# xingyizhou/CenterTrack

Hardware: AMD Instinct MI355X
Metric: frames/sec (DLA-34 + DCNv2 CenterTrack hot path: H2D of the frame + forward + decode + D2H + track association) (higher is better)
Workload: dtype f32; 1 GPU; mot17_512: mot heads, DLA-34, 512x512, 1 stream(s)/GPU, K=100, flip_test=False, seeded random-init weights; one step = 64 consecutive frames of every stream, each frame uploaded from pinned host memory inside the step (frame t+1 on a copy stream while frame t runs); global_batch=1, parallelism=streams sharded dp1, all-gather of packed detections, hip_graph=True

## Files before the change

centertrack_amd/csrc/frame_loop.hip:

```cpp
#include <stdlib.h>
#include <string.h>
#include <time.h>

#include <atomic>
#include <condition_variable>
#include <mutex>
#include <thread>
#include <vector>

#include "ct_common.h"

namespace {

class StreamPool {
public:
    explicit StreamPool(int helpers) {
        for (int i = 0; i < helpers; ++i) th_.emplace_back([this] { worker(); });
    }
    ~StreamPool() {
        {
            std::lock_guard<std::mutex> g(m_);
            stop_ = true;
            ++gen_;
        }
        cv_.notify_all();
        for (auto &t : th_) t.join();
    }
    bool run(int total, bool (*fn)(void *, int), void *ctx) {
        fn_ = fn; ctx_ = ctx; total_ = total; ok_.store(true);
        next_.store(0);
        pending_.store((int)th_.size());
        {
            std::lock_guard<std::mutex> g(m_);
            ++gen_;
        }
        cv_.notify_all();
        drain();
        while (pending_.load(std::memory_order_acquire) > 0) __builtin_ia32_pause();
        return ok_.load();
    }
private:
    void drain() {
        for (;;) {
            const int i = next_.fetch_add(1);
            if (i >= total_) break;
            if (!fn_(ctx_, i)) ok_.store(false);
        }
    }
    void worker() {
        unsigned seen = 0;
        for (;;) {
            {
                std::unique_lock<std::mutex> lk(m_);
                cv_.wait(lk, [&] { return gen_ != seen; });
                seen = gen_;
                if (stop_) return;
            }
            drain();
            pending_.fetch_sub(1, std::memory_order_release);
        }
    }
    std::vector<std::thread> th_;
    std::mutex m_;
    std::condition_variable cv_;
    unsigned gen_ = 0;
    bool stop_ = false;
    bool (*fn_)(void *, int) = nullptr;
    void *ctx_ = nullptr;
    int total_ = 0;
    std::atomic<int> next_{0}, pending_{0};
    std::atomic<bool> ok_{true};
};

struct Loop {
    ct_frame_loop_desc d;
    hipStream_t copy_stream = nullptr;
    hipEvent_t frame_ready = nullptr;
    hipEvent_t frame_done = nullptr;
    int uploaded_slot = -1;
    int pre_done_slot = -1;
    bool in_flight = false;
    int flight_slot = -1;
    StreamPool *pool = nullptr;
    ~Loop() { delete pool; }
};

struct AssocJob {
    const ct_frame_loop_desc *d;
    const float *rows, *trans_inv;
    int *counts;
    std::atomic<int> failed{-1};
    char err[256] = {0};
};

bool assoc_one(void *ctx, int b)
{
    AssocJob &j = *(AssocJob *)ctx;
    const ct_frame_loop_desc &d = *j.d;
    const int n = ct_tracker_step(d.trackers[b], j.rows + (size_t)b * d.K * d.F, d.K, d.F, &d.layout, d.out_thresh,
                                  j.trans_inv + 6 * b, d.results + (size_t)b * d.results_cap, d.results_cap);
    j.counts[b] = n;
    if (n < 0) {
        int none = -1;
        if (j.failed.compare_exchange_strong(none, b)) {
            strncpy(j.err, ct_last_error(), sizeof(j.err) - 1);
            j.err[sizeof(j.err) - 1] = 0;
        }
    }
    return n >= 0;
}

int fail(const char *what, hipError_t e)
{
    ct_set_error("%s: %s", what, hipGetErrorString(e));
    return CT_ERR_LAUNCH;
}

int prestage(Loop *L, int slot)
{
    const ct_frame_loop_desc &d = L->d;
    if (!d.pre.enabled || L->pre_done_slot == slot) return CT_OK;
    const ct_prestage_desc &p = d.pre;
    float *cur = d.frames[slot];
    const float *prev = d.frames[(slot + d.nslots - 1) % d.nslots];
    if (p.flip_B > 0) {
        const size_t half = (size_t)p.flip_B * 3 * p.H * p.W;
        int rc = ct_flip_images(cur, cur + half, (size_t)p.flip_B * 3 * p.H, p.W, d.stream);
        if (rc != CT_OK) return rc;
    }
    int rc = ct_stem_forward_parts(cur, prev, nullptr, nullptr, 0, p.N, p.H, p.W, p.w_x, p.w_img, nullptr, p.scale3, p.shift3,
                                   p.partial[slot], p.ldp, d.stream);
    if (rc != CT_OK) return rc;
    L->pre_done_slot = slot;
    return CT_OK;
}

}

extern "C" void *ct_frame_loop_create(const ct_frame_loop_desc *d)
{
    if (!d || d->B <= 0 || d->K <= 0 || d->F <= 0 || !d->trackers || !d->host_rows || !d->results || d->results_cap <= 0 ||
        d->nslots < 1 || d->nslots > 3 || d->frame_bytes == 0) {
        ct_set_error("ct_frame_loop_create: bad descriptor");
        return nullptr;
    }
    for (int i = 0; i < d->nslots; ++i)
        if (!d->graphs[i] || !d->frames[i]) {
            ct_set_error("ct_frame_loop_create: slot %d has no graph / frame buffer", i);
            return nullptr;
        }
    if (d->blob_params && (!d->blob_counts || d->blob_cap <= 0)) {
        ct_set_error("ct_frame_loop_create: blob_params without counts / capacity");
        return nullptr;
    }
    Loop *L = new Loop();
    L->d = *d;
    {
        const char *env = getenv("CENTERTRACK_HOST_THREADS");
        int threads = env ? atoi(env) : (d->B >= 8 ? (d->B / 4 < 8 ? d->B / 4 : 8) : 1);
        if (threads > d->B) threads = d->B;
        if (threads > 1) L->pool = new StreamPool(threads - 1);
    }
    hipError_t e = hipStreamCreateWithFlags(&L->copy_stream, hipStreamNonBlocking);
    if (e == hipSuccess) e = hipEventCreateWithFlags(&L->frame_ready, hipEventDisableTiming);
    if (e == hipSuccess) e = hipEventCreateWithFlags(&L->frame_done, hipEventDisableTiming);
    if (d->pre.enabled && (d->nslots != 3 || !d->pre.w_x || !d->pre.w_img || !d->pre.scale3 || !d->pre.shift3 ||
                           !d->pre.partial[0] || !d->pre.partial[1] || !d->pre.partial[2] || d->pre.ldp < 16)) {
        ct_set_error("ct_frame_loop_create: incomplete pre-stage description");
        e = hipErrorInvalidValue;
    }
    if (e != hipSuccess) {
        ct_set_error("ct_frame_loop_create: %s", hipGetErrorString(e));
        if (L->copy_stream) (void)hipStreamDestroy(L->copy_stream);
        delete L;
        return nullptr;
    }
    return L;
}

extern "C" void ct_frame_loop_destroy(void *loop)
{
    Loop *L = (Loop *)loop;
    if (!L) return;
    if (L->in_flight && L->frame_done) (void)hipEventSynchronize(L->frame_done);
    if (L->copy_stream) { (void)hipStreamSynchronize(L->copy_stream); (void)hipStreamDestroy(L->copy_stream); }
    if (L->frame_ready) (void)hipEventDestroy(L->frame_ready);
    if (L->frame_done) (void)hipEventDestroy(L->frame_done);
    delete L;
}

extern "C" int ct_frame_loop_pending_slot(void *loop) { return loop ? ((Loop *)loop)->uploaded_slot : -1; }

extern "C" int ct_frame_loop_in_flight(void *loop) { return (loop && ((Loop *)loop)->in_flight) ? ((Loop *)loop)->flight_slot : -1; }

extern "C" void ct_frame_loop_forget_upload(void *loop)
{
    Loop *L = (Loop *)loop;
    if (!L) return;
    if (L->uploaded_slot >= 0) (void)hipStreamSynchronize(L->copy_stream);
    L->uploaded_slot = -1;
    L->pre_done_slot = -1;
}

extern "C" int ct_frame_loop_prestage(void *loop, int slot)
{
    Loop *L = (Loop *)loop;
    if (!L) CT_FAIL_ARG("ct_frame_loop_prestage: null loop");
    if (slot < 0 || slot >= L->d.nslots) CT_FAIL_ARG("ct_frame_loop_prestage: slot %d of %d", slot, L->d.nslots);
    const int rc = prestage(L, slot);
    L->pre_done_slot = -1;
    return rc;
}

extern "C" int ct_frame_loop_submit(void *loop, const ct_frame_step_args *a)
{
    Loop *L = (Loop *)loop;
    if (!L || !a) CT_FAIL_ARG("ct_frame_loop_submit: null argument");
    const ct_frame_loop_desc &d = L->d;
    if (L->in_flight) CT_FAIL_ARG("ct_frame_loop_submit: the previous frame was not finished");
    if (a->slot < 0 || a->slot >= d.nslots) CT_FAIL_ARG("ct_frame_loop_submit: slot %d of %d", a->slot, d.nslots);
    hipStream_t s = (hipStream_t)d.stream;
    if (d.blob_params) {
        if (!a->trans_input) CT_FAIL_ARG("ct_frame_loop_submit: trans_input missing");
        for (int b = 0; b < d.B; ++b) {
            const int n = ct_tracker_prehm_params(d.trackers[b], d.pre_thresh, a->trans_input + 6 * b, d.inp_w, d.inp_h,
                                                  d.blob_params + (size_t)b * d.blob_cap * 3, d.blob_cap);
            if (n < 0) return CT_ERR_ARG;
            d.blob_counts[b] = n;
        }
    }
    hipError_t e = hipSuccess;
    if (a->frame_kind == CT_FRAME_UPLOADED) {
        if (L->uploaded_slot != a->slot) CT_FAIL_ARG("ct_frame_loop_submit: no upload pending for slot %d (pending: %d)", a->slot, L->uploaded_slot);
        e = hipStreamWaitEvent(s, L->frame_ready, 0);
        if (e != hipSuccess) return fail("ct_frame_loop_submit(wait for the uploaded frame)", e);
    } else if (a->frame_kind == CT_FRAME_DEVICE || a->frame_kind == CT_FRAME_HOST) {
        if (!a->frame) CT_FAIL_ARG("ct_frame_loop_submit: null frame");
        if (L->uploaded_slot >= 0) {
            e = hipStreamWaitEvent(s, L->frame_ready, 0);
            if (e != hipSuccess) return fail("ct_frame_loop_submit(wait for a stale upload)", e);
        }
        e = hipMemcpyAsync(d.frames[a->slot], a->frame, d.frame_bytes,
                           a->frame_kind == CT_FRAME_DEVICE ? hipMemcpyDeviceToDevice : hipMemcpyHostToDevice, s);
        if (e != hipSuccess) return fail("ct_frame_loop_submit(frame copy)", e);
    } else if (a->frame_kind != CT_FRAME_IN_PLACE) {
        CT_FAIL_ARG("ct_frame_loop_submit: frame_kind %d", a->frame_kind);
    }
    L->uploaded_slot = -1;
    if (a->frame_kind != CT_FRAME_UPLOADED && L->pre_done_slot == a->slot) L->pre_done_slot = -1;
    {
        const int rc = prestage(L, a->slot);
        if (rc != CT_OK) return rc;
        L->pre_done_slot = -1;
    }
    if (d.done_flag) __atomic_store_n(d.done_flag, 0, __ATOMIC_RELEASE);
    e = hipGraphLaunch((hipGraphExec_t)d.graphs[a->slot], s);
    if (e == hipSuccess) e = hipEventRecord(L->frame_done, s);
    if (e != hipSuccess) return fail("ct_frame_loop_submit(graph launch)", e);
    L->in_flight = true;
    L->flight_slot = a->slot;
    if (a->next_frame) {
        if (d.nslots < 2) CT_FAIL_ARG("ct_frame_loop_submit: uploading ahead needs >= 2 slots");
        const int ns = (a->slot + 1) % d.nslots;
        e = hipMemcpyAsync(d.frames[ns], a->next_frame, d.frame_bytes, hipMemcpyHostToDevice, L->copy_stream);
        if (e == hipSuccess) e = hipEventRecord(L->frame_ready, L->copy_stream);
        if (e != hipSuccess) return fail("ct_frame_loop_submit(upload of the next frame; the frame itself is in flight)", e);
        L->uploaded_slot = ns;
        if (d.pre.enabled) {
            e = hipStreamWaitEvent(s, L->frame_ready, 0);
            if (e != hipSuccess) return fail("ct_frame_loop_submit(pre-stage of the next frame)", e);
            const int rc = prestage(L, ns);
            if (rc != CT_OK) return rc;
        }
    }
    return CT_OK;
}

extern "C" int ct_frame_loop_upload(void *loop, int slot, const float *frame)
{
    Loop *L = (Loop *)loop;
    if (!L || !frame) CT_FAIL_ARG("ct_frame_loop_upload: null argument");
    const ct_frame_loop_desc &d = L->d;
    if (slot < 0 || slot >= d.nslots) CT_FAIL_ARG("ct_frame_loop_upload: slot %d of %d", slot, d.nslots);
    if (L->in_flight && (slot == L->flight_slot || (d.nslots == 3 && slot == (L->flight_slot + 2) % 3)))
        CT_FAIL_ARG("ct_frame_loop_upload: slot %d is read by the frame in flight", slot);
    hipError_t e = hipMemcpyAsync(d.frames[slot], frame, d.frame_bytes, hipMemcpyHostToDevice, L->copy_stream);
    if (e == hipSuccess) e = hipEventRecord(L->frame_ready, L->copy_stream);
    if (e != hipSuccess) return fail("ct_frame_loop_upload", e);
    L->uploaded_slot = slot;
    L->pre_done_slot = -1;
    if (d.pre.enabled && L->in_flight) {
        e = hipStreamWaitEvent((hipStream_t)d.stream, L->frame_ready, 0);
        if (e != hipSuccess) return fail("ct_frame_loop_upload(pre-stage)", e);
        const int rc = prestage(L, slot);
        if (rc != CT_OK) return rc;
    }
    return CT_OK;
}

extern "C" int ct_frame_loop_wait(void *loop)
{
    Loop *L = (Loop *)loop;
    if (!L) CT_FAIL_ARG("ct_frame_loop_wait: null loop");
    if (!L->in_flight) return CT_OK;
    bool seen = false;
    if (L->d.done_flag) {
        struct timespec t0, t1;
        clock_gettime(CLOCK_MONOTONIC, &t0);
        for (unsigned it = 0;; ++it) {
            if (__atomic_load_n(L->d.done_flag, __ATOMIC_ACQUIRE) == 1) { seen = true; break; }
            __builtin_ia32_pause();
            if ((it & 0x3ff) == 0x3ff) {
                clock_gettime(CLOCK_MONOTONIC, &t1);
                if ((t1.tv_sec - t0.tv_sec) * 1000000000L + (t1.tv_nsec - t0.tv_nsec) > 50000000L) break;
            }
        }
    }
    if (!seen) {
        hipError_t e = hipEventSynchronize(L->frame_done);
        if (e != hipSuccess) return fail("ct_frame_loop_wait", e);
    }
    L->in_flight = false;
    return CT_OK;
}

extern "C" int ct_frame_loop_finish(void *loop, const ct_frame_step_args *a, int *counts)
{
    Loop *L = (Loop *)loop;
    if (!L || !a || !counts) CT_FAIL_ARG("ct_frame_loop_finish: null argument");
    const ct_frame_loop_desc &d = L->d;
    if (!a->trans_inv) CT_FAIL_ARG("ct_frame_loop_finish: trans_inv missing");
    if (!L->in_flight) CT_FAIL_ARG("ct_frame_loop_finish: no frame in flight (finish follows submit exactly once)");
    int rc = ct_frame_loop_wait(loop);
    if (rc != CT_OK) return rc;
    const float *rows = d.host_rows;
    if (d.rows_keep) {
        memcpy(d.rows_keep, d.host_rows, sizeof(float) * (size_t)d.B * d.K * d.F);
        rows = d.rows_keep;
    }
    AssocJob job;
    job.d = &d; job.rows = rows; job.trans_inv = a->trans_inv; job.counts = counts;
    bool ok = true;
    if (L->pool) {
        ok = L->pool->run(d.B, assoc_one, &job);
    } else {
        for (int b = 0; b < d.B; ++b) ok = assoc_one(&job, b) && ok;
    }
    if (!ok) {
        ct_set_error("ct_frame_loop_finish: ct_tracker_step failed for stream %d: %s", job.failed.load(), job.err);
        return CT_ERR_ARG;
    }
    return CT_OK;
}

extern "C" int ct_frame_loop_finish_submit(void *loop, const ct_frame_step_args *cur, int *counts, const ct_frame_step_args *next)
{
    int rc = ct_frame_loop_finish(loop, cur, counts);
    if (rc != CT_OK) return rc;
    return ct_frame_loop_submit(loop, next);
}
```

Baseline: 1154 frames/s.

## Run next-frame pre-stage on a separate low-priority stream after frame completes

Moves the pre-stage for the next frame (optional flip plus the partial stem convolution over the current and previous frames) off the main compute stream onto a dedicated low-priority stream. By default it is deferred until the host sees the in-flight frame finish, then issued on the side stream. The next submit waits on a pre_done event instead of redoing the work or waiting on the upload. The goal is to stop the pre-stage from being serialized inside the main stream between graph launches and from competing with the running forward pass. The cost is extra events, cross-stream waits and more complex slot-state bookkeeping. With the default flag trigger, the pre-stage starts only after the host notices completion, so it may add latency before the next launch.

```diff
diff --git a/centertrack_amd/csrc/frame_loop.hip b/centertrack_amd/csrc/frame_loop.hip
--- a/centertrack_amd/csrc/frame_loop.hip
+++ b/centertrack_amd/csrc/frame_loop.hip
@@ -77,6 +77,11 @@
     hipStream_t copy_stream = nullptr;
     hipEvent_t frame_ready = nullptr;
     hipEvent_t frame_done = nullptr;
+    hipStream_t pre_stream = nullptr;
+    hipEvent_t pre_done = nullptr;
+    hipEvent_t frame_in = nullptr;
+    bool trigger_upload = false, trigger_flag = true;
+    int pre_wait_slot = -1;
     int uploaded_slot = -1;
     int pre_done_slot = -1;
     bool in_flight = false;
@@ -116,22 +121,39 @@
     return CT_ERR_LAUNCH;
 }
 
-int prestage(Loop *L, int slot)
+int prestage(Loop *L, int slot, hipStream_t stream)
 {
     const ct_frame_loop_desc &d = L->d;
-    if (!d.pre.enabled || L->pre_done_slot == slot) return CT_OK;
+    if (!d.pre.enabled) return CT_OK;
     const ct_prestage_desc &p = d.pre;
     float *cur = d.frames[slot];
     const float *prev = d.frames[(slot + d.nslots - 1) % d.nslots];
     if (p.flip_B > 0) {
         const size_t half = (size_t)p.flip_B * 3 * p.H * p.W;
-        int rc = ct_flip_images(cur, cur + half, (size_t)p.flip_B * 3 * p.H, p.W, d.stream);
+        int rc = ct_flip_images(cur, cur + half, (size_t)p.flip_B * 3 * p.H, p.W, stream);
         if (rc != CT_OK) return rc;
     }
     int rc = ct_stem_forward_parts(cur, prev, nullptr, nullptr, 0, p.N, p.H, p.W, p.w_x, p.w_img, nullptr, p.scale3, p.shift3,
-                                   p.partial[slot], p.ldp, d.stream);
+                                   p.partial[slot], p.ldp, stream);
     if (rc != CT_OK) return rc;
     L->pre_done_slot = slot;
+    return CT_OK;
+}
+
+int prestage_ahead(Loop *L, int slot, bool frame_ended = false)
+{
+    if (L->pre_done_slot == slot) return CT_OK;
+    if (L->trigger_flag && !frame_ended) {
+        L->pre_wait_slot = slot;
+        return CT_OK;
+    }
+    hipError_t e = hipStreamWaitEvent(L->pre_stream, L->frame_ready, 0);
+    if (e == hipSuccess && !frame_ended) e = hipStreamWaitEvent(L->pre_stream, L->trigger_upload ? L->frame_in : L->frame_done, 0);
+    if (e != hipSuccess) return fail("pre-stage of the next frame (wait)", e);
+    const int rc = prestage(L, slot, L->pre_stream);
+    if (rc != CT_OK) return rc;
+    e = hipEventRecord(L->pre_done, L->pre_stream);
+    if (e != hipSuccess) { L->pre_done_slot = -1; return fail("pre-stage of the next frame (record)", e); }
     return CT_OK;
 }
 
@@ -160,10 +182,22 @@
         int threads = env ? atoi(env) : (d->B >= 8 ? (d->B / 4 < 8 ? d->B / 4 : 8) : 1);
         if (threads > d->B) threads = d->B;
         if (threads > 1) L->pool = new StreamPool(threads - 1);
+        const char *trig = getenv("CENTERTRACK_PRESTAGE_TRIGGER");
+        L->trigger_upload = trig && strcmp(trig, "upload") == 0;
+        L->trigger_flag = !trig || (strcmp(trig, "upload") != 0 && strcmp(trig, "frame") != 0);
     }
     hipError_t e = hipStreamCreateWithFlags(&L->copy_stream, hipStreamNonBlocking);
     if (e == hipSuccess) e = hipEventCreateWithFlags(&L->frame_ready, hipEventDisableTiming);
     if (e == hipSuccess) e = hipEventCreateWithFlags(&L->frame_done, hipEventDisableTiming);
+    if (e == hipSuccess && d->pre.enabled) {
+        int least = 0, greatest = 0;
+        e = hipDeviceGetStreamPriorityRange(&least, &greatest);
+        const char *prio = getenv("CENTERTRACK_PRESTAGE_PRIORITY");
+        if (prio && strcmp(prio, "normal") == 0) least = 0;
+        if (e == hipSuccess) e = hipStreamCreateWithPriority(&L->pre_stream, hipStreamNonBlocking, least);
+        if (e == hipSuccess) e = hipEventCreateWithFlags(&L->pre_done, hipEventDisableTiming);
+        if (e == hipSuccess) e = hipEventCreateWithFlags(&L->frame_in, hipEventDisableTiming);
+    }
     if (d->pre.enabled && (d->nslots != 3 || !d->pre.w_x || !d->pre.w_img || !d->pre.scale3 || !d->pre.shift3 ||
                            !d->pre.partial[0] || !d->pre.partial[1] || !d->pre.partial[2] || d->pre.ldp < 16)) {
         ct_set_error("ct_frame_loop_create: incomplete pre-stage description");
@@ -172,6 +206,11 @@
     if (e != hipSuccess) {
         ct_set_error("ct_frame_loop_create: %s", hipGetErrorString(e));
         if (L->copy_stream) (void)hipStreamDestroy(L->copy_stream);
+        if (L->pre_stream) (void)hipStreamDestroy(L->pre_stream);
+        if (L->frame_ready) (void)hipEventDestroy(L->frame_ready);
+        if (L->frame_done) (void)hipEventDestroy(L->frame_done);
+        if (L->pre_done) (void)hipEventDestroy(L->pre_done);
+        if (L->frame_in) (void)hipEventDestroy(L->frame_in);
         delete L;
         return nullptr;
     }
@@ -184,8 +223,11 @@
     if (!L) return;
     if (L->in_flight && L->frame_done) (void)hipEventSynchronize(L->frame_done);
     if (L->copy_stream) { (void)hipStreamSynchronize(L->copy_stream); (void)hipStreamDestroy(L->copy_stream); }
+    if (L->pre_stream) { (void)hipStreamSynchronize(L->pre_stream); (void)hipStreamDestroy(L->pre_stream); }
     if (L->frame_ready) (void)hipEventDestroy(L->frame_ready);
     if (L->frame_done) (void)hipEventDestroy(L->frame_done);
+    if (L->pre_done) (void)hipEventDestroy(L->pre_done);
+    if (L->frame_in) (void)hipEventDestroy(L->frame_in);
     delete L;
 }
 
@@ -198,6 +240,8 @@
     Loop *L = (Loop *)loop;
     if (!L) return;
     if (L->uploaded_slot >= 0) (void)hipStreamSynchronize(L->copy_stream);
+    if (L->pre_stream) (void)hipStreamSynchronize(L->pre_stream);
+    L->pre_wait_slot = -1;
     L->uploaded_slot = -1;
     L->pre_done_slot = -1;
 }
@@ -207,7 +251,13 @@
     Loop *L = (Loop *)loop;
     if (!L) CT_FAIL_ARG("ct_frame_loop_prestage: null loop");
     if (slot < 0 || slot >= L->d.nslots) CT_FAIL_ARG("ct_frame_loop_prestage: slot %d of %d", slot, L->d.nslots);
-    const int rc = prestage(L, slot);
+    int rc = CT_OK;
+    if (L->pre_done_slot == slot) {
+        const hipError_t e = hipStreamWaitEvent((hipStream_t)L->d.stream, L->pre_done, 0);
+        if (e != hipSuccess) rc = fail("ct_frame_loop_prestage(wait for the pre-stage)", e);
+    } else {
+        rc = prestage(L, slot, (hipStream_t)L->d.stream);
+    }
     L->pre_done_slot = -1;
     return rc;
 }
@@ -232,7 +282,7 @@
     hipError_t e = hipSuccess;
     if (a->frame_kind == CT_FRAME_UPLOADED) {
         if (L->uploaded_slot != a->slot) CT_FAIL_ARG("ct_frame_loop_submit: no upload pending for slot %d (pending: %d)", a->slot, L->uploaded_slot);
-        e = hipStreamWaitEvent(s, L->frame_ready, 0);
+        if (L->pre_done_slot != a->slot) e = hipStreamWaitEvent(s, L->frame_ready, 0);
         if (e != hipSuccess) return fail("ct_frame_loop_submit(wait for the uploaded frame)", e);
     } else if (a->frame_kind == CT_FRAME_DEVICE || a->frame_kind == CT_FRAME_HOST) {
         if (!a->frame) CT_FAIL_ARG("ct_frame_loop_submit: null frame");
@@ -240,6 +290,10 @@
             e = hipStreamWaitEvent(s, L->frame_ready, 0);
             if (e != hipSuccess) return fail("ct_frame_loop_submit(wait for a stale upload)", e);
         }
+        if (L->pre_done_slot >= 0) {
+            e = hipStreamWaitEvent(s, L->pre_done, 0);
+            if (e != hipSuccess) return fail("ct_frame_loop_submit(wait for a stale pre-stage)", e);
+        }
         e = hipMemcpyAsync(d.frames[a->slot], a->frame, d.frame_bytes,
                            a->frame_kind == CT_FRAME_DEVICE ? hipMemcpyDeviceToDevice : hipMemcpyHostToDevice, s);
         if (e != hipSuccess) return fail("ct_frame_loop_submit(frame copy)", e);
@@ -247,11 +301,21 @@
         CT_FAIL_ARG("ct_frame_loop_submit: frame_kind %d", a->frame_kind);
     }
     L->uploaded_slot = -1;
+    L->pre_wait_slot = -1;
     if (a->frame_kind != CT_FRAME_UPLOADED && L->pre_done_slot == a->slot) L->pre_done_slot = -1;
-    {
-        const int rc = prestage(L, a->slot);
-        if (rc != CT_OK) return rc;
+    if (d.pre.enabled) {
+        if (L->pre_done_slot == a->slot) {
+            e = hipStreamWaitEvent(s, L->pre_done, 0);
+            if (e != hipSuccess) return fail("ct_frame_loop_submit(wait for the pre-stage)", e);
+        } else {
+            const int rc = prestage(L, a->slot, s);
+            if (rc != CT_OK) return rc;
+        }
         L->pre_done_slot = -1;
+        if (L->trigger_upload) {
+            e = hipEventRecord(L->frame_in, s);
+            if (e != hipSuccess) return fail("ct_frame_loop_submit(frame_in)", e);
+        }
     }
     if (d.done_flag) __atomic_store_n(d.done_flag, 0, __ATOMIC_RELEASE);
     e = hipGraphLaunch((hipGraphExec_t)d.graphs[a->slot], s);
@@ -267,9 +331,7 @@
         if (e != hipSuccess) return fail("ct_frame_loop_submit(upload of the next frame; the frame itself is in flight)", e);
         L->uploaded_slot = ns;
         if (d.pre.enabled) {
-            e = hipStreamWaitEvent(s, L->frame_ready, 0);
-            if (e != hipSuccess) return fail("ct_frame_loop_submit(pre-stage of the next frame)", e);
-            const int rc = prestage(L, ns);
+            const int rc = prestage_ahead(L, ns);
             if (rc != CT_OK) return rc;
         }
     }
@@ -284,15 +346,16 @@
     if (slot < 0 || slot >= d.nslots) CT_FAIL_ARG("ct_frame_loop_upload: slot %d of %d", slot, d.nslots);
     if (L->in_flight && (slot == L->flight_slot || (d.nslots == 3 && slot == (L->flight_slot + 2) % 3)))
         CT_FAIL_ARG("ct_frame_loop_upload: slot %d is read by the frame in flight", slot);
-    hipError_t e = hipMemcpyAsync(d.frames[slot], frame, d.frame_bytes, hipMemcpyHostToDevice, L->copy_stream);
+    hipError_t e = hipSuccess;
+    if (L->pre_done_slot >= 0) e = hipStreamWaitEvent(L->copy_stream, L->pre_done, 0);
+    if (e == hipSuccess) e = hipMemcpyAsync(d.frames[slot], frame, d.frame_bytes, hipMemcpyHostToDevice, L->copy_stream);
     if (e == hipSuccess) e = hipEventRecord(L->frame_ready, L->copy_stream);
     if (e != hipSuccess) return fail("ct_frame_loop_upload", e);
     L->uploaded_slot = slot;
     L->pre_done_slot = -1;
+    L->pre_wait_slot = -1;
     if (d.pre.enabled && L->in_flight) {
-        e = hipStreamWaitEvent((hipStream_t)d.stream, L->frame_ready, 0);
-        if (e != hipSuccess) return fail("ct_frame_loop_upload(pre-stage)", e);
-        const int rc = prestage(L, slot);
+        const int rc = prestage_ahead(L, slot);
         if (rc != CT_OK) return rc;
     }
     return CT_OK;
@@ -321,6 +384,11 @@
         if (e != hipSuccess) return fail("ct_frame_loop_wait", e);
     }
     L->in_flight = false;
+    if (L->pre_wait_slot >= 0) {
+        const int slot = L->pre_wait_slot;
+        L->pre_wait_slot = -1;
+        if (slot == L->uploaded_slot) return prestage_ahead(L, slot, true);
+    }
     return CT_OK;
 }
 
```

Result: no change. 1152 frames/s (median of 3 runs) (-0.2%).
